# DoubangoTelecom/compv

Measured on AMD Instinct MI355X. Metric: Mpixels/s Sobel->Canny->HoughSHT on 4K uint8, higher is better.
Workload: dtype u8; 1 GPU; batched 3840x2160 uint8 frames, Sobel3x3 -> Canny(59,119) -> HoughSHT(rho=1, theta=1deg, thr=100); 256 distinct frames resident per GPU as 8 batches of 32, a step processes one batch, steps rotate over the batches; frames_per_gpu=32, resident_batches=8, parallelism=frames sharded across 1 GPU(s), no data-path collective

## Files before the change

### compv_amd/capi.py

```python
import ctypes as C
import importlib.util
import os

import numpy as np

_HERE = os.path.dirname(os.path.abspath(__file__))
LIB_PATH = os.path.join(_HERE, "lib", "libcompv_hip.so")

OK = 0
E_NOT_IMPLEMENTED = -1
E_NOT_INITIALIZED = -2
E_INVALID_STATE = -3
E_INVALID_PARAMETER = -4
E_OUT_OF_MEMORY = -5
E_OUT_OF_BOUND = -6
E_HIP = -7

OP_SOBEL, OP_SCHARR, OP_PREWITT = 0, 2, 3
THRESHOLD_COMPARE_TO_GRADIENT, THRESHOLD_PERCENT_OF_MEAN, THRESHOLD_OTSU = 0, 1, 2
(FMT_RGBA32, FMT_ARGB32, FMT_BGRA32, FMT_RGB24, FMT_BGR24, FMT_RGB565LE, FMT_RGB565BE, FMT_BGR565LE, FMT_BGR565BE,
 FMT_YUYV422, FMT_UYVY422, FMT_Y) = range(12)
FMT_BYTES = [4, 4, 4, 3, 3, 2, 2, 2, 2, 2, 2, 1]
FMT_NV12, FMT_NV21, FMT_YUV420P, FMT_YUV422P, FMT_YUV444P, FMT_HSV = range(12, 18)
MORPH_ERODE, MORPH_DILATE, MORPH_OPEN, MORPH_CLOSE = 0, 1, 2, 3
# ... 11 lines not shown
HOMOGRAPHY_RESULT_DTYPE = np.dtype([("H", "<f8", (9,)), ("variance", "<f8"), ("inliers", "<i4"), ("bestTry", "<i4"), ("status", "<i4"), ("rotations", "<i4")])
CURVEFIT_LINE, CURVEFIT_PARABOLA, CURVEFIT_PARABOLA_SIDEWAYS = 0, 1, 2
SVM_KERNEL_LINEAR, SVM_KERNEL_RBF = 0, 2
SVM_F32, SVM_F64 = 0, 1
UNDISTORT_F32, UNDISTORT_F64 = 0, 1
UNDISTORT_COEFFS = 14
MOMENTS_VALUE, MOMENTS_UNIT = 0, 1
MOMENTS_ORIGIN_FRAME, MOMENTS_ORIGIN_BOX = 0, 1
MOMENTS_DTYPE = np.dtype([(k, "<u8") for k in ("m00", "m01", "m10", "m11", "m02", "m20")])
MOMENTS_SHAPE_DTYPE = np.dtype([(k, "<f8") for k in ("xbar", "ybar", "u20", "u02", "u11", "skew", "cs", "sn")] + [("status", "<i4"), ("pad", "<i4")])
CURVEFIT_RESULT_DTYPE = np.dtype([("A", "<f8"), ("B", "<f8"), ("C", "<f8"), ("inliers", "<i4"), ("bestTry", "<i4"), ("status", "<i4"), ("k", "<i4")])

EXPORTS = [
    "compvhip_device_count", "compvhip_ctx_create", "compvhip_ctx_destroy", "compvhip_last_error",
    "compvhip_live_allocations", "compvhip_debug_alloc_fill", "compvhip_edge_dete_u8", "compvhip_canny_u8", "compvhip_houghsht_u8",
    "compvhip_houghsht_dims", "compvhip_houghsht_vote_grid", "compvhip_plan_create", "compvhip_plan_destroy", "compvhip_plan_canny",
    "compvhip_plan_houghsht", "compvhip_plan_pipeline", "compvhip_plan_acc", "compvhip_plan_edge_counts",
    "compvhip_plan_set_timing", "compvhip_plan_get_timing", "compvhip_plan_acc_export", "compvhip_plan_edge_dete",
    "compvhip_houghkht_u8", "compvhip_grayscale_u8", "compvhip_otsu_u8", "compvhip_plan_grayscale", "compvhip_plan_otsu",
    "compvhip_gauss_kernel_fixedpoint", "compvhip_convlt1_fixedpoint_u8", "compvhip_plan_convlt1_fixedpoint", "compvhip_plan_to_cartesian",
    "compvhip_plan_pipeline_async", "compvhip_plan_wait", "compvhip_houghsht_to_cartesian", "compvhip_houghkht_to_cartesian",
    "compvhip_houghkht_kernels_u8", "compvhip_houghkht_stage_ms", "compvhip_convlt1_8u16s16s", "compvhip_convlt1_16s16s16s",
    "compvhip_plan_pipeline_ex", "compvhip_plan_houghkht", "compvhip_plan_houghkht_stage_ms", "compvhip_houghkht_link_u8",
    "compvhip_houghkht_dims", "compvhip_host_cpu_budget", "compvhip_plan_houghkht_ex", "compvhip_houghkht_ex_u8",
    "compvhip_plan_houghsht_segments", "compvhip_houghsht_segments_u8",
    "compvhip_plan_houghsht_fit", "compvhip_houghsht_fit_u8",
    "compvhip_plan_components", "compvhip_components_u8",
    "compvhip_threshold_u8", "compvhip_plan_threshold", "compvhip_threshold_adaptive_u8", "compvhip_plan_threshold_adaptive",
    "compvhip_morph_strel", "compvhip_morph_u8", "compvhip_plan_morph", "compvhip_plan_morph_ex",
    "compvhip_plan_fast", "compvhip_fast_u8",
    "compvhip_plan_orb_keypoints", "compvhip_plan_orb_describe", "compvhip_orb_u8",
# ... 1520 lines not shown
def host_cpu_budget():
    lib = load()
    lib.compvhip_host_cpu_budget.restype = C.c_int
    return int(lib.compvhip_host_cpu_budget())


def houghsht_vote_grid(W, H, theta_deg=1.0, frames=1):
    lib = load()
    nx = C.c_int(0); ny = C.c_int(0); rw = C.c_int(0)
    rc = lib.compvhip_houghsht_vote_grid(W, H, theta_deg, frames, C.byref(nx), C.byref(ny), C.byref(rw))
    if rc:
        raise CompvHipError(rc, "compvhip_houghsht_vote_grid")
    return nx.value, ny.value, rw.value


def houghkht_dims(W, H, rho=1.0, theta_deg=1.0):
    lib = load()
    r = C.c_size_t(0); t = C.c_size_t(0)
    lib.compvhip_houghkht_dims.argtypes = [C.c_size_t, C.c_size_t, C.c_float, C.c_float, C.POINTER(C.c_size_t), C.POINTER(C.c_size_t)]
    rc = lib.compvhip_houghkht_dims(W, H, rho, theta_deg, C.byref(r), C.byref(t))
    if rc:
        raise CompvHipError(rc, "compvhip_houghkht_dims")
    return int(t.value), int(r.value)


def to_cartesian(W, H, lines, kht=False):
    L = load()
    n = len(lines)
    buf = np.zeros(max(n, 1), LINE_DTYPE)
    for i, l in enumerate(lines):
# ... 25 lines not shown
```

### compv_amd/csrc/api.cpp

```cpp
#include "api_internal.hpp"

namespace {
__attribute__((noinline, optnone)) float libmCosf(float x) { return cosf(x); }
__attribute__((noinline, optnone)) float libmSinf(float x) { return sinf(x); }

void gradientThresholds(float fLow, float fHigh, int* tLow, int* tHigh)
{
	const float l = fLow < 1.f ? 1.f : (fLow > 65535.f ? 65535.f : fLow);
	const float h = fHigh < 1.f ? 1.f : (fHigh > 65535.f ? 65535.f : fHigh);
	uint16_t lo = static_cast<uint16_t>(l), hi = static_cast<uint16_t>(h);
	lo = static_cast<uint16_t>(std::max<int>(1, lo));
	hi = static_cast<uint16_t>(std::max<int>(lo + 2, hi));
	*tLow = lo; *tHigh = hi;
}

void cannyCoverage(size_t W, int* simdEnd, int* cStart)
{
	const size_t maxCols = W - 1;
	size_t mpw = 1;
	if (maxCols >= 16) mpw = 16; else if (maxCols >= 8) mpw = 8;
	if (mpw == 1) { *simdEnd = 1; *cStart = 1; return; }
	size_t col = 1;
	while (col + (mpw - 1) < maxCols) col += mpw;
	*simdEnd = static_cast<int>(col);
// ... 11 lines not shown
	float tt = 0.f;
	for (size_t t = 0; t < T; ++t, tt += fTheta) {
		sinQ[t] = static_cast<int32_t>((libmSinf(tt) * fRho) * 65535.f);
		cosQ[t] = static_cast<int32_t>((libmCosf(tt) * fRho) * 65535.f);
	}
}

static size_t voteMaxWindow()
{
	const char* e = getenv("COMPVHIP_VOTE_MAX_WINDOW");
	const long n = e ? atol(e) : 0;
	return (n >= 64 && n <= kShtMaxWindow) ? static_cast<size_t>(n) : static_cast<size_t>(kShtMaxWindow);
}

static bool voteGridTables(size_t W, size_t H, const std::vector<int32_t>& sinQ, const std::vector<int32_t>& cosQ, int split, int& nx, int& ny, int& TW, int& TH, long long& worst,
                           std::vector<int32_t>* kt, std::vector<int32_t>* rowBase)
{
	const size_t T = sinQ.size();
	const long long barrier = static_cast<long long>(W + H);
	nx = 1; ny = 1;
	for (int k = 0; k < split; ++k) {
		const double tw = static_cast<double>(W) / nx, th = static_cast<double>(H) / ny;
		if (tw >= th) ++nx; else ++ny;
	}
	TW = static_cast<int>(alignUp((W + nx - 1) / nx, 32)); TH = static_cast<int>((H + ny - 1) / ny);
	nx = static_cast<int>((W + TW - 1) / TW);
	const int tiles = nx * ny;
	if (kt) { kt->assign(static_cast<size_t>(tiles) * T, 0); rowBase->assign(static_cast<size_t>(tiles) * T, 0); }
	worst = 0;
	for (int ty = 0; ty < ny; ++ty) for (int tx = 0; tx < nx; ++tx) {
		const long long x0 = static_cast<long long>(tx) * TW, y0 = static_cast<long long>(ty) * TH;
		const long long mx = TW - 1, my = TH - 1;
		for (size_t t = 0; t < T; ++t) {
			const long long c = cosQ[t], sn = sinQ[t];
			const long long C = x0 * c + y0 * sn;
			long long Chi = C / 65536; if (C - Chi * 65536 < 0) --Chi;
			const long long Clo = C - Chi * 65536;
			const long long corners[4] = { Clo, mx * c + Clo, my * sn + Clo, mx * c + my * sn + Clo };
			long long qmin = 0, qmax = 0;
			for (int k = 0; k < 4; ++k) {
				long long q = corners[k] / 65536; if (corners[k] - q * 65536 < 0) --q;
				if (k == 0 || q < qmin) qmin = q;
				if (k == 0 || q > qmax) qmax = q;
			}
			const long long base = barrier - Chi - qmax;
			const long long d = ((base % 16) + 16) % 16;
			worst = std::max(worst, qmax - qmin + 1 + d);
			if (kt) {
				(*kt)[(static_cast<size_t>(ty) * nx + tx) * T + t] = static_cast<int32_t>((qmax + d) * 65536 + 65535 - Clo);
				(*rowBase)[(static_cast<size_t>(ty) * nx + tx) * T + t] = static_cast<int32_t>(base - d);
			}
		}
	}
	return alignUp(static_cast<size_t>(worst), 16) <= voteMaxWindow() && TW <= 1280 &&
	       static_cast<long long>(TW - 1) * 65535 + static_cast<long long>(TH - 1) * 65535 < 0x7f000000LL;
}

bool planVoteTiles(size_t W, size_t H, size_t frames, const std::vector<int32_t>& sinQ, const std::vector<int32_t>& cosQ, ShtTileArgs& v, std::vector<int32_t>& kt,
                   std::vector<int32_t>& rowBase)
{
	const size_t T = sinQ.size();
	const int groups = static_cast<int>((T + 63) / 64);
	int first = -1;
	for (int split = 0; split < 512 && first < 0; ++split) {
		int nx, ny, TW, TH; long long worst;
		if (voteGridTables(W, H, sinQ, cosQ, split, nx, ny, TW, TH, worst, nullptr, nullptr)) first = split;
	}
	if (first < 0) return false;
	int best = first; double bestCost = 0.0;
	int nx0, ny0, TW0, TH0; long long worst0;
	(void)voteGridTables(W, H, sinQ, cosQ, first, nx0, ny0, TW0, TH0, worst0, nullptr, nullptr);
	const bool starved = static_cast<double>(frames) * nx0 * ny0 * groups < 64.0;
	for (int split = first; starved && split <= first + 4; ++split) {
		int nx, ny, TW, TH; long long worst;
		if (!voteGridTables(W, H, sinQ, cosQ, split, nx, ny, TW, TH, worst, nullptr, nullptr)) continue;
		const double rw = static_cast<double>(alignUp(static_cast<size_t>(worst), 16));
		const double wgs = static_cast<double>(frames) * nx * ny * groups;
		const double rounds = wgs <= 1024.0 ? std::ceil(wgs / 256.0) : wgs / 256.0;
		const double perWg = 67.0 * (static_cast<double>(TW) * TH) / (960.0 * 720.0) + 9.3 * rw / 1208.0;
		const double reduce = 36.0 * (static_cast<double>(frames) * nx * ny * rw) / (32.0 * 12.0 * 1208.0);
		const double cost = rounds * perWg + reduce;
		if (split == first || cost < bestCost * 0.97) { best = split; bestCost = cost; }
	}
	int nx, ny, TW, TH; long long worst;
	if (!voteGridTables(W, H, sinQ, cosQ, best, nx, ny, TW, TH, worst, &kt, &rowBase)) return false;
	v.nx = nx; v.ny = ny; v.TW = TW; v.TH = TH; v.tiles = nx * ny;
	v.Rw = static_cast<int>(alignUp(static_cast<size_t>(worst), 16)); v.rwPitch = v.Rw;
	v.groups = groups; v.Tpad = v.groups * 64;
	v.tileCap = static_cast<size_t>(TW) * TH;
	return true;
}

ShtArgs shtArgs(compvhip_plan* p, int threshold)
{
	ShtArgs a;
	a.ebits = p->ebits; a.edges = p->edges; a.edgeCounts = p->edgeCounts; a.acc = p->acc;
	a.sinQ = p->sinQ; a.cosQ = p->cosQ; a.lineKeys = p->keysA; a.lineVals = p->valsA; a.lineCounts = p->lineCounts;
	a.frameTotals = p->frameTotals; a.lineTotal = p->lineTotal; a.sortN = 0; a.outCounts = nullptr; a.stepFlags = nullptr; a.hostStep = nullptr;
	a.nmsRange = p->nmsRange; a.blockCounts = p->blockCounts; a.lineBlocks = p->lineBlocks; a.nmsFlags = p->nmsFlags; a.nmsRows = static_cast<int>(sht_nms_rows(static_cast<int>(p->R))); a.nmsGroups = sht_nms_groups(static_cast<int>(p->T));
	a.bitsFrameStride = p->bitsFrameStride; a.edgeCap = p->edgeCap; a.accFrameStride = p->accFrameStride; a.lineCap = p->lineCap;
// ... 116 lines not shown
	{
		std::vector<float> ct(T), ist(T);
		for (size_t t = 0; t < T; ++t) {
			const float theta = static_cast<float>(t) * step;
			ct[t] = libmCosf(theta);
			ist[t] = 1.f / libmSinf(theta);
		}
		HIPCHK(ctx, p->cosT.reserve(ctx, T));
		HIPCHK(ctx, p->invSinT.reserve(ctx, T));
		HIPCHK(ctx, hipMemcpy(p->cosT, ct.data(), T * sizeof(float), hipMemcpyHostToDevice));
		HIPCHK(ctx, hipMemcpy(p->invSinT, ist.data(), T * sizeof(float), hipMemcpyHostToDevice));
	}
	{
		if (p->vt.tiles <= 0 || p->vtKt.size() != static_cast<size_t>(p->vt.tiles) * T) return fail(ctx, COMPVHIP_E_INVALID_STATE, "vote tiles were not planned");
		{
			const int tiles = p->vt.tiles, Rw = p->vt.Rw, groups = sht_nms_groups(static_cast<int>(T));
			std::vector<int2> range(static_cast<size_t>(groups));
			for (int g = 0; g < groups; ++g) {
				int lo = INT32_MAX, hi = INT32_MIN;
				for (int c = 8 * g - 1; c <= 8 * g + 8; ++c) {
					if (c < 0 || c >= static_cast<int>(T)) continue;
					for (int i = 0; i < tiles; ++i) {
						const int b = p->vtRowBase[static_cast<size_t>(i) * T + c];
						lo = std::min(lo, b); hi = std::max(hi, b + Rw);
					}
				}
				range[g] = make_int2(lo - 1, hi + 1);
			}
			std::vector<int2> reach(T);
			for (size_t t = 0; t < T; ++t) {
				int lo = INT32_MAX, hi = INT32_MIN;
				for (int i = 0; i < tiles; ++i) {
					const int b = p->vtRowBase[static_cast<size_t>(i) * T + t];
					lo = std::min(lo, b); hi = std::max(hi, b + Rw);
				}
				reach[t] = make_int2(lo, hi);
			}
			HIPCHK(ctx, p->reach.reserve(ctx, reach.size()));
			HIPCHK(ctx, hipMemcpy(p->reach, reach.data(), reach.size() * sizeof(int2), hipMemcpyHostToDevice));
			HIPCHK(ctx, p->nmsRange.reserve(ctx, range.size()));
			HIPCHK(ctx, hipMemcpy(p->nmsRange, range.data(), range.size() * sizeof(int2), hipMemcpyHostToDevice));
		}
		HIPCHK(ctx, p->dKt.reserve(ctx, p->vtKt.size()));
		HIPCHK(ctx, p->dRowBase.reserve(ctx, p->vtRowBase.size()));
		HIPCHK(ctx, hipMemcpy(p->dKt, p->vtKt.data(), p->vtKt.size() * sizeof(int32_t), hipMemcpyHostToDevice));
		HIPCHK(ctx, hipMemcpy(p->dRowBase, p->vtRowBase.data(), p->vtRowBase.size() * sizeof(int32_t), hipMemcpyHostToDevice));
		{
			const size_t cols = p->frames * p->vt.tiles * static_cast<size_t>(p->vt.Tpad);
			HIPCHK(ctx, p->partLo.reserve(ctx, cols * p->vt.rwPitch));
			HIPCHK(ctx, p->partHi.reserve(ctx, cols * p->vt.rwPitch));
			HIPCHK(ctx, p->colFlag.reserve(ctx, cols));
		}
		p->vt.kt = p->dKt; p->vt.rowBase = p->dRowBase; p->vt.partLo = p->partLo; p->vt.partHi = p->partHi; p->vt.colFlag = p->colFlag; p->vt.reach = p->reach; p->vt.tileCounts = p->tileCounts;
		p->edgeCap = static_cast<size_t>(p->vt.tiles) * p->vt.tileCap;
	}
	HIPCHK(ctx, p->edges.reserve(ctx, p->edgeCap * p->frames));
	HIPCHK(ctx, p->acc.reserve(ctx, p->accFrameStride * p->frames));
	HIPCHK(ctx, hipMemset(p->acc, 0, sizeof(uint16_t) * p->accFrameStride * p->frames));
	p->strengthBits = 1;
	while ((static_cast<size_t>(1) << p->strengthBits) <= 2 * (p->W > p->H ? p->W : p->H)) p->strengthBits++;
	if (p->strengthBits > 16) p->strengthBits = 16;
	int frameBits = 0;
	while ((static_cast<size_t>(1) << frameBits) < p->frames) frameBits++;
	p->keyBits = frameBits + p->strengthBits;
	if (R * T >= (static_cast<size_t>(1) << 32)) return fail(ctx, COMPVHIP_E_INVALID_PARAMETER, "theta step too small: the accumulator has 2^32 cells or more");
	if (p->keyBits > 32) return fail(ctx, COMPVHIP_E_INVALID_PARAMETER, "too many frames for a 32-bit line key");
// ... 118 lines not shown
		if (theta == 0.f) { out[0] = rho + halfW; out[1] = r; out[2] = rho + halfW; out[3] = -r; continue; }
		const float c = libmCosf(theta) * halfW, inv = 1.f / libmSinf(theta);
		out[0] = 0.f; out[1] = ((rho + c) * inv) + halfH;
		out[2] = widthF; out[3] = ((rho - c) * inv) + halfH;
	}
	return COMPVHIP_OK;
}

int compvhip_houghsht_vote_grid(size_t W, size_t H, float thetaDeg, size_t frames, int* nx, int* ny, int* windowRows)
{
	size_t R = 0, T = 0; float st = 0.f;
	if (!nx || !ny || !windowRows || !frames) return COMPVHIP_E_INVALID_PARAMETER;
	const int rc = shtDims(W, H, thetaDeg, &R, &T, &st);
	if (rc) return rc;
	if (T < 5) return COMPVHIP_E_NOT_IMPLEMENTED;
	std::vector<int32_t> sq, cq, kt, rb;
	shtTables(thetaDeg, T, sq, cq);
	ShtTileArgs v = {};
	if (!planVoteTiles(W, H, frames, sq, cq, v, kt, rb)) return COMPVHIP_E_NOT_IMPLEMENTED;
	*nx = v.nx; *ny = v.ny; *windowRows = v.Rw;
	return COMPVHIP_OK;
}

int compvhip_host_cpu_budget(void)
{
	return static_cast<int>(std::min<size_t>(hostCpuBudget(), 0x7fffffff));
}

int compvhip_houghsht_dims(size_t W, size_t H, float thetaDeg, size_t* R, size_t* T, float* step)
{
	if (!R || !T) return COMPVHIP_E_INVALID_PARAMETER;
	return shtDims(W, H, thetaDeg, R, T, step);
}

int compvhip_houghkht_dims(size_t W, size_t H, float rho, float thetaDeg, size_t* rhoN, size_t* T)
// ... 18 lines not shown
	p->tilesY = static_cast<int>((H + 63) / 64);
	p->wb = p->tilesX * 16;
	p->bitsFrameStride = static_cast<size_t>(p->wb) * H;
	auto failed = [&](int rc) { compvhip_plan_destroy(p); return fail(ctx, rc, "plan allocation"); };
	if (p->ebits.reserve(ctx, p->bitsFrameStride * frames) != hipSuccess) return failed(COMPVHIP_E_OUT_OF_MEMORY);
	if (p->ubits.reserve(ctx, p->bitsFrameStride * frames) != hipSuccess) return failed(COMPVHIP_E_OUT_OF_MEMORY);
	if (hipMemset(p->ebits, 0, sizeof(uint32_t) * p->bitsFrameStride * frames) != hipSuccess) return failed(COMPVHIP_E_HIP);
	if (hipMemset(p->ubits, 0, sizeof(uint32_t) * p->bitsFrameStride * frames) != hipSuccess) return failed(COMPVHIP_E_HIP);
	if (hipDeviceSynchronize() != hipSuccess) return failed(COMPVHIP_E_HIP);
	{
		p->voteTiles = true;
		size_t R = 0, T = 0; float step = 0.f;
		if (p->voteTiles && shtDims(W, H, thetaDeg, &R, &T, &step) == COMPVHIP_OK && T >= 5) {
			std::vector<int32_t> sq, cq;
			shtTables(thetaDeg, T, sq, cq);
			if (!planVoteTiles(W, H, frames, sq, cq, p->vt, p->vtKt, p->vtRowBase)) p->voteTiles = false;
		}
		else p->voteTiles = false;
		p->lineBlocks = p->voteTiles ? sht_lines_blocks(static_cast<int>(R)) : 0;
		p->nCounts = (2 + static_cast<size_t>(p->voteTiles ? p->vt.tiles : 0) + static_cast<size_t>(p->lineBlocks)) * frames + (frames + 1) * kFrameSlot;
	}
	if (p->counters.reserve(ctx, p->nCounts + kMaxRounds) != hipSuccess) return failed(COMPVHIP_E_OUT_OF_MEMORY);
	p->edgeCounts = p->counters; p->lineCounts = p->counters + frames; p->tileCounts = p->counters + 2 * frames; p->blockCounts = p->counters + (2 + static_cast<size_t>(p->voteTiles ? p->vt.tiles : 0)) * frames; p->flags = p->counters + p->nCounts;
	p->frameTotals = p->blockCounts + static_cast<size_t>(p->lineBlocks) * frames; p->lineTotal = reinterpret_cast<unsigned int*>(p->frameTotals + frames * kFrameSlot);
	if (const char* e = getenv("COMPVHIP_RESOLVE_WRAP")) { const int v = atoi(e); if (v >= 8 && v <= kMaxRounds && (v & 3) == 0) p->maxRounds = v; }
	p->traceRounds = getenv("COMPVHIP_TRACE_ROUNDS") != nullptr;
	if (hipMemset(p->counters, 0, sizeof(int) * (p->nCounts + kMaxRounds)) != hipSuccess) return failed(COMPVHIP_E_HIP);
	if (p->thrDev.reserve(ctx, frames) != hipSuccess) return failed(COMPVHIP_E_OUT_OF_MEMORY);
	if (p->dirty.reserve(ctx, canny_resolve_dirty_bytes(static_cast<int>(H), p->wb, static_cast<int>(frames))) != hipSuccess) return failed(COMPVHIP_E_OUT_OF_MEMORY);
	if (p->sums.reserve(ctx, frames * kFrameSlot) != hipSuccess) return failed(COMPVHIP_E_OUT_OF_MEMORY);
	if (p->hFlags.reserve(2) != hipSuccess) return failed(COMPVHIP_E_OUT_OF_MEMORY);
// ... 482 lines not shown
```

### compv_amd/csrc/api_internal.hpp

```cpp
#pragma once
#include "../../include/compv_hip.h"
#include "kernels.hpp"
#include "kht.hpp"
#include "kht_group.hpp"
#include "device_memory.hpp"
#include "host_call.hpp"
#include "frame_slices.hpp"
#include "convert_math.hpp"
#include "step_policy.hpp"

#include <hip/hip_runtime.h>

#include <algorithm>
#include <atomic>
#include <chrono>
#include <cmath>
#include <cstdio>
#include <cstdlib>
#include <cstring>
#include <functional>
#include <memory>
#include <string>
#include <thread>
#include <type_traits>
// ... 156 lines not shown
	DevBuf<uint8_t> nmsFlags;
	int* blockCounts = nullptr; int lineBlocks = 0;
	DevBuf<uint8_t> sortTemp; size_t sortTempBytes = 0;
	DevBuf<int32_t> segPerLine;
	DevBuf<int32_t> compRows; DevBuf<uint32_t> compBits; DevBuf<int32_t> compParent;
	DevBuf<uint8_t> morphTmp;
	DevBuf<int> fastWork; DevBuf<uint8_t> fastScores;
	DevBuf<int32_t> orbIndex; DevBuf<uint8_t> orbBlur; uint16_t orbKern[5] = {}; bool orbKernReady = false; bool orbBriefLds = false;
	WarpTables warp;
	DevBuf<float> hogCells;
	StatsScratch stats;
	int strengthBits = 16, keyBits = 0;
	DevBuf<uint16_t> chunkHist; DevBuf<uint32_t> strengthStart; int sortChunks = 0; bool deviceSort = false;
	bool voteTiles = false;
	ShtTileArgs vt = {};
	std::vector<int32_t> vtKt, vtRowBase;
	DevBuf<int32_t> dKt, dRowBase; DevBuf<uint8_t> partLo, partHi, colFlag; int* tileCounts = nullptr;
	std::vector<std::unique_ptr<KhtGroupState>> khtBatch;
	std::vector<std::unique_ptr<KhtPeaksWork>> khtWork;
	double khtStageMs[6] = {}; double khtWallMs = 0.0; int khtThreads = 0;
	struct AsyncStep { bool used = false; bool replay = false; uint64_t seq = 0; hipEvent_t done = nullptr; hipStream_t stream = nullptr; StepParams sp; size_t sortN = 0; int rounds = 0; } steps[kAsyncDepth];
	uint64_t stepSeq = 0;
};

struct compvhip_matcher : TimingState {
	compvhip_ctx* ctx = nullptr;
	int descDwords = 0, queryCap = 0, trainCap = 0, pairs = 0, knn = 0;
	DevBuf<uint32_t> partial;
	DevBuf<compvhip_match> reverse;
};
struct RansacHandle : TimingState {
	compvhip_ctx* ctx = nullptr;
// ... 233 lines not shown
```

### compv_amd/csrc/kernels.hpp

```cpp
#pragma once
#include <hip/hip_runtime.h>
#include <stddef.h>
#include <stdint.h>

#include "../../include/compv_hip.h"

namespace compvhip {

#ifndef COMPVHIP_BAND_H
#define COMPVHIP_BAND_H 64
#endif
constexpr int kBandH = COMPVHIP_BAND_H;
#ifndef COMPVHIP_BAND_WORDS
#define COMPVHIP_BAND_WORDS 64
#endif
constexpr int kBandWords = COMPVHIP_BAND_WORDS;
constexpr int kResolveThreads = 512;
constexpr int kFrameSlot = 32;
constexpr int kResolveRows = kBandH * kBandWords / kResolveThreads;

struct CannyArgs {
	const uint8_t* in;
	uint8_t* out;
	uint32_t* ebits;
// ... 96 lines not shown
	const int* stepFlags;
	int* hostStep;
	int32_t* outCounts;
	int* frameTotals;
	unsigned int* lineTotal;
	size_t sortN;
	size_t bitsFrameStride, edgeCap, accFrameStride, lineCap;
	int W, H, wb;
	int R, T, accPitch, barrier;
	int threshold, nmsLastCol;
	int frames;
	int strengthBits;
};
struct ShtTileArgs {
	const int32_t* kt;
	const int32_t* rowBase;
	uint8_t* partLo;
	uint8_t* partHi;
	uint8_t* colFlag;
	const int2* reach;
	int* tileCounts;
	int nx, ny, TW, TH, tiles;
	int Rw, rwPitch;
	int Tpad, groups;
	size_t tileCap;
};
constexpr int kShtMaxWindow = 1264;
hipError_t launch_sht_compact_tiles(const ShtArgs& a, const ShtTileArgs& v, int frames, hipStream_t stream);
hipError_t launch_sht_vote_tiles(const ShtArgs& a, const ShtTileArgs& v, int frames, hipStream_t stream);
hipError_t launch_sht_reduce_tiles(const ShtArgs& a, const ShtTileArgs& v, int frames, hipStream_t stream);
hipError_t launch_bytes_to_bits(const uint8_t* edges, int W, int H, int S, size_t frameStride, uint32_t* ebits, int wb, size_t bitsFrameStride,
// ... 478 lines not shown
```

### compv_amd/csrc/sht_tiles_kernels.hip

```cpp
#include "device.hpp"

namespace compvhip {

constexpr int kTcThreads = 256;
constexpr int kTcRows = 64;
constexpr int kTcStage = 6144;

__global__ __launch_bounds__(kTcThreads) void sht_compact_tiles_kernel(ShtArgs a, ShtTileArgs v)
{
	__shared__ int s_wave[kTcThreads / 64];
	__shared__ int s_base;
	__shared__ uint32_t s_stage[kTcStage];
	const int frame = blockIdx.y;
	const int chunksPerTile = (v.TH + kTcRows - 1) / kTcRows;
	const int tile = blockIdx.x / chunksPerTile, chunk = blockIdx.x - tile * chunksPerTile;
	const int ty = tile / v.nx, tx = tile - ty * v.nx;
	const int x0 = tx * v.TW, y0 = ty * v.TH;
	const int wpr = v.TW >> 5;
	const uint32_t wprInv = (1u << 20) / (uint32_t)wpr + 1u;
	const int ly0 = chunk * kTcRows;
	const int rows = min(min(kTcRows, v.TH - ly0), a.H - (y0 + ly0));
	const int nwords = max(rows, 0) * wpr;
	const uint32_t* __restrict__ bits = a.ebits + (size_t)frame * a.bitsFrameStride;
	const int w0 = x0 >> 5;
// ... 51 lines not shown
	size_t pos = (size_t)s_base + first;
#pragma unroll
	for (int k = 0; k < kPer; ++k) {
		uint32_t b = wv[k];
		while (b) {
			const int bit = __ffs(b) - 1;
			b &= b - 1;
			if (pos < v.tileCap) dst[pos] = (uint32_t)(wl[k] + bit);
			++pos;
		}
	}
}

constexpr int kVtThreads = 1024;
constexpr int kVtUnroll = 32;

__global__ __launch_bounds__(kVtThreads) void sht_vote_tiles_kernel(ShtArgs a, ShtTileArgs v)
{
	extern __shared__ __attribute__((aligned(16))) uint32_t hist[];
	const int units = a.frames * v.tiles;
	const int xcd = blockIdx.x & 7, k = blockIdx.x >> 3;
	const int g = k % v.groups;
	const int unit = (k / v.groups) * 8 + xcd;
	if (unit >= units) return;
	const int frame = unit / v.tiles, tile = unit - frame * v.tiles;
	const int tid = threadIdx.x, lane = tid & 63;
	const int wave = __builtin_amdgcn_readfirstlane(tid >> 6);

	const int nAll = v.tileCounts[unit];
	if (g == 0 && threadIdx.x == 0 && nAll) atomicAdd(&a.edgeCounts[frame], nAll);
	const int n = min(nAll, (int)v.tileCap);
	const int words = v.Rw * 32;
	uint32_t* const s_any = hist + words;
	if (tid < 2) s_any[tid] = 0u;
	for (int i = tid * 4; i < words; i += kVtThreads * 4) *reinterpret_cast<uint4*>(&hist[i]) = make_uint4(0, 0, 0, 0);

	const int t = g * 64 + lane;
	const int tt = min(t, a.T - 1);
	const int nc = -a.cosQ[tt], ns = -a.sinQ[tt];
	const int K = v.kt[(size_t)tile * a.T + tt];
	uint32_t inc = (t < a.T) ? ((lane & 32) ? 0x10000u : 1u) : 0u;
	asm volatile("" : "+v"(inc));
	const uint32_t lane4 = (uint32_t)(lane & 31) * 4u;
	__syncthreads();

	const uint32_t* __restrict__ list = a.edges + (size_t)unit * v.tileCap;
	typedef uint32_t u32x16 __attribute__((ext_vector_type(16)));
	auto vote = [&](uint32_t e) {
		const int lx = (int)(e & 0xffffu), ly = (int)(e >> 16);
		int val, ad;
		asm volatile("v_mad_i32_i24 %0, %1, %2, %3" : "=v"(val) : "s"(lx), "v"(nc), "v"(K));
		asm volatile("v_mad_i32_i24 %0, %1, %2, %3" : "=v"(val) : "s"(ly), "v"(ns), "v"(val));
		const uint32_t row = (uint32_t)val >> 16;
		asm volatile("v_lshl_add_u32 %0, %1, 7, %2" : "=v"(ad) : "v"(row), "v"(lane4));
		asm volatile("ds_add_u32 %0, %1" : : "v"(ad), "v"(inc) : "memory");
	};
	const int nblk = n / kVtUnroll;
	constexpr int kStep = kVtThreads / 64;
// ... 16 lines not shown
			VT_VOTE(b0, b1);
			if (b >= nblk) break;
			VT_WAIT(a0, a1);
		}
	}
#undef VT_LOAD
#undef VT_WAIT
#undef VT_VOTE
	for (int i = nblk * kVtUnroll + wave; i < n; i += kStep) vote(__builtin_amdgcn_readfirstlane(list[i]));
	__builtin_amdgcn_s_waitcnt(0xc07f);
	__syncthreads();

	const size_t column = ((size_t)unit * v.Tpad) + (size_t)g * 64 + lane;
	uint8_t* __restrict__ partLo = v.partLo + column * v.rwPitch;
	uint8_t* __restrict__ partHi = v.partHi + column * v.rwPitch;
	const uint32_t sel1 = (lane & 32) ? 0x07030602u : 0x05010400u;
	typedef uint32_t u32x4 __attribute__((ext_vector_type(4)));
	auto bytes16 = [&](int w0, u32x4& lo, u32x4& hi) {
		uint32_t h[16];
#pragma unroll
		for (int j = 0; j < 16; ++j) h[j] = hist[(w0 + j) * 32 + (lane & 31)];
#pragma unroll
		for (int q = 0; q < 4; ++q) {
			const uint32_t p01 = __builtin_amdgcn_perm(h[4 * q + 1], h[4 * q], sel1), p23 = __builtin_amdgcn_perm(h[4 * q + 3], h[4 * q + 2], sel1);
			lo[q] = __builtin_amdgcn_perm(p23, p01, 0x05040100u);
			hi[q] = __builtin_amdgcn_perm(p23, p01, 0x07060302u);
		}
	};
	uint32_t any = 0u;
	for (int wb = wave * 128; wb < v.Rw; wb += (kVtThreads / 64) * 128)
	for (int w0 = wb; w0 < min(wb + 128, v.Rw); w0 += 16) {
		u32x4 lo, hi;
		bytes16(w0, lo, hi);
		any |= hi.x | hi.y | hi.z | hi.w;
		uint8_t* const dst = partLo + w0;
		asm volatile("global_store_dwordx4 %0, %1, off" : : "v"(dst), "v"(lo) : "memory");
	}
	const uint64_t mine = __ballot(any != 0u);
	if (lane == 0 && mine) { atomicOr(&s_any[0], (uint32_t)mine); atomicOr(&s_any[1], (uint32_t)(mine >> 32)); }
	__syncthreads();
	const uint32_t m0 = s_any[0], m1 = s_any[1];
	const bool flagged = (((lane & 32) ? m1 : m0) >> (lane & 31)) & 1u;
	if (wave == 0) v.colFlag[column] = flagged ? 1 : 0;
	if ((m0 | m1) == 0u) return;
	if (flagged) {
		for (int wb = wave * 128; wb < v.Rw; wb += (kVtThreads / 64) * 128)
		for (int w0 = wb; w0 < min(wb + 128, v.Rw); w0 += 16) {
			u32x4 lo, hi;
			bytes16(w0, lo, hi);
			uint8_t* const dst = partHi + w0;
			asm volatile("global_store_dwordx4 %0, %1, off" : : "v"(dst), "v"(hi) : "memory");
		}
	}
}

constexpr int kRdThreads = 64;
constexpr int kRdRows = 16;

__global__ __launch_bounds__(kRdThreads) void sht_reduce_tiles_kernel(ShtArgs a, ShtTileArgs v)
{
	const int frame = blockIdx.z, theta = blockIdx.y;
	const int2 reach = v.reach[theta];
	if ((int)(blockIdx.x * kRdThreads * kRdRows) >= reach.y || (int)((blockIdx.x + 1) * kRdThreads * kRdRows) <= reach.x) return;
	const int r0 = (blockIdx.x * kRdThreads + threadIdx.x) * kRdRows;
	if (r0 >= a.accPitch) return;
	uint32_t E[4] = { 0, 0, 0, 0 }, O[4] = { 0, 0, 0, 0 };
	int covers = 0;
	for (int tile = 0; tile < v.tiles; ++tile) {
		const int base = v.rowBase[(size_t)tile * a.T + theta];
		const int w0 = r0 - base;
		if (w0 < 0 || w0 >= v.Rw) continue;
		++covers;
		const size_t column = ((size_t)frame * v.tiles + tile) * v.Tpad + theta;
		const uint4 c = *reinterpret_cast<const uint4*>(v.partLo + column * v.rwPitch + w0);
		E[0] += c.x & 0x00ff00ffu; O[0] += (c.x >> 8) & 0x00ff00ffu;
		E[1] += c.y & 0x00ff00ffu; O[1] += (c.y >> 8) & 0x00ff00ffu;
		E[2] += c.z & 0x00ff00ffu; O[2] += (c.z >> 8) & 0x00ff00ffu;
		E[3] += c.w & 0x00ff00ffu; O[3] += (c.w >> 8) & 0x00ff00ffu;
		if (v.colFlag[column]) {
			const uint4 h = *reinterpret_cast<const uint4*>(v.partHi + column * v.rwPitch + w0);
			E[0] += (h.x & 0x00ff00ffu) << 8; O[0] += h.x & 0xff00ff00u;
			E[1] += (h.y & 0x00ff00ffu) << 8; O[1] += h.y & 0xff00ff00u;
			E[2] += (h.z & 0x00ff00ffu) << 8; O[2] += h.z & 0xff00ff00u;
			E[3] += (h.w & 0x00ff00ffu) << 8; O[3] += h.w & 0xff00ff00u;
		}
	}
// ... 50 lines not shown
```

### include/compv_hip.h

```cpp
#ifndef COMPV_HIP_H
#define COMPV_HIP_H

#include <stddef.h>
#include <stdint.h>

#ifdef __cplusplus
extern "C" {
#endif

#if defined(__GNUC__)
#	define COMPVHIP_API __attribute__((visibility("default")))
#else
#	define COMPVHIP_API
#endif

enum {
	COMPVHIP_OK = 0,
	COMPVHIP_E_NOT_IMPLEMENTED = -1,
	COMPVHIP_E_NOT_INITIALIZED = -2,
	COMPVHIP_E_INVALID_STATE = -3,
	COMPVHIP_E_INVALID_PARAMETER = -4,
	COMPVHIP_E_OUT_OF_MEMORY = -5,
	COMPVHIP_E_OUT_OF_BOUND = -6,
	COMPVHIP_E_HIP = -7
// ... 68 lines not shown
                                      compvhip_line* lines, size_t cap, size_t* n, double* gs);

COMPVHIP_API int compvhip_houghkht_kernels_u8(compvhip_ctx* ctx, const uint8_t* edges, size_t W, size_t H, size_t S,
                                              double clusterMinDeviation, size_t clusterMinSize,
                                              double* kernels7, size_t cap, size_t* n, double* hmax);
COMPVHIP_API int compvhip_houghkht_stage_ms(compvhip_ctx* ctx, double* ms6);
COMPVHIP_API int compvhip_houghkht_link_u8(const uint8_t* edges, size_t W, size_t H, size_t S, size_t clusterMinSize, int32_t* xy, size_t cap, size_t* nPoints,
                                           uint32_t* stringEnds, size_t stringCap, size_t* nStrings);

COMPVHIP_API int compvhip_houghsht_to_cartesian(size_t W, size_t H, const compvhip_line* lines, size_t n, float* out);
COMPVHIP_API int compvhip_houghkht_to_cartesian(size_t W, size_t H, const compvhip_line* lines, size_t n, float* out);

COMPVHIP_API int compvhip_houghsht_dims(size_t W, size_t H, float thetaDeg, size_t* R, size_t* T, float* thetaStepRad);
COMPVHIP_API int compvhip_houghkht_dims(size_t W, size_t H, float rho, float thetaDeg, size_t* rhoN, size_t* T);
COMPVHIP_API int compvhip_houghsht_vote_grid(size_t W, size_t H, float thetaDeg, size_t frames, int* nx, int* ny, int* windowRows);
COMPVHIP_API int compvhip_host_cpu_budget(void);


COMPVHIP_API int compvhip_plan_create(compvhip_ctx* ctx, size_t W, size_t H, size_t S, size_t frames, float thetaDeg,
                                      compvhip_plan** plan);
COMPVHIP_API void compvhip_plan_destroy(compvhip_plan* plan);

COMPVHIP_API int compvhip_plan_canny(compvhip_plan* plan, const uint8_t* d_in, float tLow, float tHigh, int ksize,
                                     int thresholdType, uint8_t* d_edges, void* stream);

COMPVHIP_API int compvhip_plan_grayscale(compvhip_plan* plan, const uint8_t* d_in, int pixfmt, uint8_t* d_gray, void* stream);

COMPVHIP_API int compvhip_plan_otsu(compvhip_plan* plan, const uint8_t* d_gray, int32_t* d_thresholds, void* stream);

COMPVHIP_API int compvhip_plan_convlt1_fixedpoint(compvhip_plan* plan, const uint8_t* d_in, const uint16_t* vtKern, const uint16_t* hzKern,
// ... 504 lines not shown
```

Measured before the change: 437,000 Mpixels/s.

## Limit SHT vote flush to per-column row reach and reuse histogram bytes

Records a per-tile, per-theta row reach and packs it alongside rowBase as int2, so the vote kernel writes only the rows each column can actually receive instead of the full worst-case window Rw. The flush now reads each histogram tile once with a permlane32 swap and keeps the high bytes in registers, rather than rereading for the partHi pass. The reduction kernel bounds its reads by the per-column reach, and the partial buffers are zeroed at plan time so rows never written read as zero. It also adds a host export for the vote tables; a fixed per-wave flush count of 5 is assumed, which risks missing rows if the reach exceeds 16*5*16 rows.

```diff
diff --git a/compv_amd/capi.py b/compv_amd/capi.py
--- a/compv_amd/capi.py
+++ b/compv_amd/capi.py
@@ -49,7 +49,7 @@
 EXPORTS = [
     "compvhip_device_count", "compvhip_ctx_create", "compvhip_ctx_destroy", "compvhip_last_error",
     "compvhip_live_allocations", "compvhip_debug_alloc_fill", "compvhip_edge_dete_u8", "compvhip_canny_u8", "compvhip_houghsht_u8",
-    "compvhip_houghsht_dims", "compvhip_houghsht_vote_grid", "compvhip_plan_create", "compvhip_plan_destroy", "compvhip_plan_canny",
+    "compvhip_houghsht_dims", "compvhip_houghsht_vote_grid", "compvhip_houghsht_vote_tables", "compvhip_plan_create", "compvhip_plan_destroy", "compvhip_plan_canny",
     "compvhip_plan_houghsht", "compvhip_plan_pipeline", "compvhip_plan_acc", "compvhip_plan_edge_counts",
     "compvhip_plan_set_timing", "compvhip_plan_get_timing", "compvhip_plan_acc_export", "compvhip_plan_edge_dete",
     "compvhip_houghkht_u8", "compvhip_grayscale_u8", "compvhip_otsu_u8", "compvhip_plan_grayscale", "compvhip_plan_otsu",
@@ -1600,6 +1600,23 @@
     return nx.value, ny.value, rw.value
 
 
+def houghsht_vote_tables(W, H, theta_deg=1.0, frames=1):
+    lib = load()
+    nx, ny, rw = houghsht_vote_grid(W, H, theta_deg, frames)
+    r = C.c_size_t(0); t = C.c_size_t(0)
+    lib.compvhip_houghsht_dims(W, H, theta_deg, C.byref(r), C.byref(t), None)
+    T = t.value
+    tw = C.c_int(0); th = C.c_int(0)
+    cq, sq = np.zeros(T, np.int32), np.zeros(T, np.int32)
+    kt, rb, rr = (np.zeros((nx * ny, T), np.int32) for _ in range(3))
+    i32 = C.POINTER(C.c_int32)
+    lib.compvhip_houghsht_vote_tables.argtypes = [C.c_size_t, C.c_size_t, C.c_float, C.c_size_t, C.POINTER(C.c_int), C.POINTER(C.c_int), i32, i32, i32, i32, i32, C.c_size_t]
+    rc = lib.compvhip_houghsht_vote_tables(W, H, theta_deg, frames, C.byref(tw), C.byref(th), *(a.ctypes.data_as(i32) for a in (cq, sq, kt, rb, rr)), kt.size)
+    if rc:
+        raise CompvHipError(rc, "compvhip_houghsht_vote_tables")
+    return {"nx": nx, "ny": ny, "rw": rw, "TW": tw.value, "TH": th.value, "cosQ": cq, "sinQ": sq, "K": kt, "rowBase": rb, "rowReach": rr}
+
+
 def houghkht_dims(W, H, rho=1.0, theta_deg=1.0):
     lib = load()
     r = C.c_size_t(0); t = C.c_size_t(0)
diff --git a/compv_amd/csrc/api.cpp b/compv_amd/csrc/api.cpp
--- a/compv_amd/csrc/api.cpp
+++ b/compv_amd/csrc/api.cpp
@@ -49,7 +49,7 @@
 }
 
 static bool voteGridTables(size_t W, size_t H, const std::vector<int32_t>& sinQ, const std::vector<int32_t>& cosQ, int split, int& nx, int& ny, int& TW, int& TH, long long& worst,
-                           std::vector<int32_t>* kt, std::vector<int32_t>* rowBase)
+                           std::vector<int32_t>* kt, std::vector<int32_t>* rowBase, std::vector<int32_t>* rowReach)
 {
 	const size_t T = sinQ.size();
 	const long long barrier = static_cast<long long>(W + H);
@@ -61,7 +61,7 @@
 	TW = static_cast<int>(alignUp((W + nx - 1) / nx, 32)); TH = static_cast<int>((H + ny - 1) / ny);
 	nx = static_cast<int>((W + TW - 1) / TW);
 	const int tiles = nx * ny;
-	if (kt) { kt->assign(static_cast<size_t>(tiles) * T, 0); rowBase->assign(static_cast<size_t>(tiles) * T, 0); }
+	if (kt) { kt->assign(static_cast<size_t>(tiles) * T, 0); rowBase->assign(static_cast<size_t>(tiles) * T, 0); rowReach->assign(static_cast<size_t>(tiles) * T, 0); }
 	worst = 0;
 	for (int ty = 0; ty < ny; ++ty) for (int tx = 0; tx < nx; ++tx) {
 		const long long x0 = static_cast<long long>(tx) * TW, y0 = static_cast<long long>(ty) * TH;
@@ -84,6 +84,7 @@
 			if (kt) {
 				(*kt)[(static_cast<size_t>(ty) * nx + tx) * T + t] = static_cast<int32_t>((qmax + d) * 65536 + 65535 - Clo);
 				(*rowBase)[(static_cast<size_t>(ty) * nx + tx) * T + t] = static_cast<int32_t>(base - d);
+				(*rowReach)[(static_cast<size_t>(ty) * nx + tx) * T + t] = static_cast<int32_t>(alignUp(static_cast<size_t>(qmax - qmin + 1 + d), 16));
 			}
 		}
 	}
@@ -92,23 +93,23 @@
 }
 
 bool planVoteTiles(size_t W, size_t H, size_t frames, const std::vector<int32_t>& sinQ, const std::vector<int32_t>& cosQ, ShtTileArgs& v, std::vector<int32_t>& kt,
-                   std::vector<int32_t>& rowBase)
+                   std::vector<int32_t>& rowBase, std::vector<int32_t>& rowReach)
 {
 	const size_t T = sinQ.size();
 	const int groups = static_cast<int>((T + 63) / 64);
 	int first = -1;
 	for (int split = 0; split < 512 && first < 0; ++split) {
 		int nx, ny, TW, TH; long long worst;
-		if (voteGridTables(W, H, sinQ, cosQ, split, nx, ny, TW, TH, worst, nullptr, nullptr)) first = split;
+		if (voteGridTables(W, H, sinQ, cosQ, split, nx, ny, TW, TH, worst, nullptr, nullptr, nullptr)) first = split;
 	}
 	if (first < 0) return false;
 	int best = first; double bestCost = 0.0;
 	int nx0, ny0, TW0, TH0; long long worst0;
-	(void)voteGridTables(W, H, sinQ, cosQ, first, nx0, ny0, TW0, TH0, worst0, nullptr, nullptr);
+	(void)voteGridTables(W, H, sinQ, cosQ, first, nx0, ny0, TW0, TH0, worst0, nullptr, nullptr, nullptr);
 	const bool starved = static_cast<double>(frames) * nx0 * ny0 * groups < 64.0;
 	for (int split = first; starved && split <= first + 4; ++split) {
 		int nx, ny, TW, TH; long long worst;
-		if (!voteGridTables(W, H, sinQ, cosQ, split, nx, ny, TW, TH, worst, nullptr, nullptr)) continue;
+		if (!voteGridTables(W, H, sinQ, cosQ, split, nx, ny, TW, TH, worst, nullptr, nullptr, nullptr)) continue;
 		const double rw = static_cast<double>(alignUp(static_cast<size_t>(worst), 16));
 		const double wgs = static_cast<double>(frames) * nx * ny * groups;
 		const double rounds = wgs <= 1024.0 ? std::ceil(wgs / 256.0) : wgs / 256.0;
@@ -118,7 +119,7 @@
 		if (split == first || cost < bestCost * 0.97) { best = split; bestCost = cost; }
 	}
 	int nx, ny, TW, TH; long long worst;
-	if (!voteGridTables(W, H, sinQ, cosQ, best, nx, ny, TW, TH, worst, &kt, &rowBase)) return false;
+	if (!voteGridTables(W, H, sinQ, cosQ, best, nx, ny, TW, TH, worst, &kt, &rowBase, &rowReach)) return false;
 	v.nx = nx; v.ny = ny; v.TW = TW; v.TH = TH; v.tiles = nx * ny;
 	v.Rw = static_cast<int>(alignUp(static_cast<size_t>(worst), 16)); v.rwPitch = v.Rw;
 	v.groups = groups; v.Tpad = v.groups * 64;
@@ -265,27 +266,24 @@
 	{
 		if (p->vt.tiles <= 0 || p->vtKt.size() != static_cast<size_t>(p->vt.tiles) * T) return fail(ctx, COMPVHIP_E_INVALID_STATE, "vote tiles were not planned");
 		{
-			const int tiles = p->vt.tiles, Rw = p->vt.Rw, groups = sht_nms_groups(static_cast<int>(T));
+			const int tiles = p->vt.tiles, groups = sht_nms_groups(static_cast<int>(T));
+			std::vector<int2> reach(T);
+			for (size_t t = 0; t < T; ++t) {
+				int lo = INT32_MAX, hi = INT32_MIN;
+				for (int i = 0; i < tiles; ++i) {
+					const int b = p->vtRowBase[static_cast<size_t>(i) * T + t];
+					lo = std::min(lo, b); hi = std::max(hi, b + p->vtRowReach[static_cast<size_t>(i) * T + t]);
+				}
+				reach[t] = make_int2(lo, hi);
+			}
 			std::vector<int2> range(static_cast<size_t>(groups));
 			for (int g = 0; g < groups; ++g) {
 				int lo = INT32_MAX, hi = INT32_MIN;
 				for (int c = 8 * g - 1; c <= 8 * g + 8; ++c) {
 					if (c < 0 || c >= static_cast<int>(T)) continue;
-					for (int i = 0; i < tiles; ++i) {
-						const int b = p->vtRowBase[static_cast<size_t>(i) * T + c];
-						lo = std::min(lo, b); hi = std::max(hi, b + Rw);
-					}
+					lo = std::min(lo, reach[static_cast<size_t>(c)].x); hi = std::max(hi, reach[static_cast<size_t>(c)].y);
 				}
 				range[g] = make_int2(lo - 1, hi + 1);
-			}
-			std::vector<int2> reach(T);
-			for (size_t t = 0; t < T; ++t) {
-				int lo = INT32_MAX, hi = INT32_MIN;
-				for (int i = 0; i < tiles; ++i) {
-					const int b = p->vtRowBase[static_cast<size_t>(i) * T + t];
-					lo = std::min(lo, b); hi = std::max(hi, b + Rw);
-				}
-				reach[t] = make_int2(lo, hi);
 			}
 			HIPCHK(ctx, p->reach.reserve(ctx, reach.size()));
 			HIPCHK(ctx, hipMemcpy(p->reach, reach.data(), reach.size() * sizeof(int2), hipMemcpyHostToDevice));
@@ -293,14 +291,24 @@
 			HIPCHK(ctx, hipMemcpy(p->nmsRange, range.data(), range.size() * sizeof(int2), hipMemcpyHostToDevice));
 		}
 		HIPCHK(ctx, p->dKt.reserve(ctx, p->vtKt.size()));
-		HIPCHK(ctx, p->dRowBase.reserve(ctx, p->vtRowBase.size()));
 		HIPCHK(ctx, hipMemcpy(p->dKt, p->vtKt.data(), p->vtKt.size() * sizeof(int32_t), hipMemcpyHostToDevice));
-		HIPCHK(ctx, hipMemcpy(p->dRowBase, p->vtRowBase.data(), p->vtRowBase.size() * sizeof(int32_t), hipMemcpyHostToDevice));
+		{
+			const size_t Tpad = static_cast<size_t>(p->vt.Tpad);
+			std::vector<int2> rb(static_cast<size_t>(p->vt.tiles) * Tpad, make_int2(0, 0));
+			for (size_t i = 0; i < static_cast<size_t>(p->vt.tiles); ++i)
+				for (size_t t = 0; t < T; ++t) rb[i * Tpad + t] = make_int2(p->vtRowBase[i * T + t], p->vtRowReach[i * T + t]);
+			HIPCHK(ctx, p->dRowBase.reserve(ctx, rb.size()));
+			HIPCHK(ctx, hipMemcpy(p->dRowBase, rb.data(), rb.size() * sizeof(int2), hipMemcpyHostToDevice));
+		}
 		{
 			const size_t cols = p->frames * p->vt.tiles * static_cast<size_t>(p->vt.Tpad);
 			HIPCHK(ctx, p->partLo.reserve(ctx, cols * p->vt.rwPitch));
 			HIPCHK(ctx, p->partHi.reserve(ctx, cols * p->vt.rwPitch));
 			HIPCHK(ctx, p->colFlag.reserve(ctx, cols));
+			HIPCHK(ctx, hipMemset(p->partLo, 0, cols * p->vt.rwPitch));
+			HIPCHK(ctx, hipMemset(p->partHi, 0, cols * p->vt.rwPitch));
+			HIPCHK(ctx, hipMemset(p->colFlag, 0, cols));
+			HIPCHK(ctx, hipDeviceSynchronize());
 		}
 		p->vt.kt = p->dKt; p->vt.rowBase = p->dRowBase; p->vt.partLo = p->partLo; p->vt.partHi = p->partHi; p->vt.colFlag = p->colFlag; p->vt.reach = p->reach; p->vt.tileCounts = p->tileCounts;
 		p->edgeCap = static_cast<size_t>(p->vt.tiles) * p->vt.tileCap;
@@ -449,11 +457,30 @@
 	const int rc = shtDims(W, H, thetaDeg, &R, &T, &st);
 	if (rc) return rc;
 	if (T < 5) return COMPVHIP_E_NOT_IMPLEMENTED;
-	std::vector<int32_t> sq, cq, kt, rb;
+	std::vector<int32_t> sq, cq, kt, rb, rr;
 	shtTables(thetaDeg, T, sq, cq);
 	ShtTileArgs v = {};
-	if (!planVoteTiles(W, H, frames, sq, cq, v, kt, rb)) return COMPVHIP_E_NOT_IMPLEMENTED;
+	if (!planVoteTiles(W, H, frames, sq, cq, v, kt, rb, rr)) return COMPVHIP_E_NOT_IMPLEMENTED;
 	*nx = v.nx; *ny = v.ny; *windowRows = v.Rw;
+	return COMPVHIP_OK;
+}
+
+int compvhip_houghsht_vote_tables(size_t W, size_t H, float thetaDeg, size_t frames, int* TW, int* TH, int32_t* cosQ, int32_t* sinQ, int32_t* kt, int32_t* rowBase,
+                                  int32_t* rowReach, size_t cap)
+{
+	size_t R = 0, T = 0; float st = 0.f;
+	if (!TW || !TH || !cosQ || !sinQ || !kt || !rowBase || !rowReach || !frames) return COMPVHIP_E_INVALID_PARAMETER;
+	const int rc = shtDims(W, H, thetaDeg, &R, &T, &st);
+	if (rc) return rc;
+	if (T < 5) return COMPVHIP_E_NOT_IMPLEMENTED;
+	std::vector<int32_t> sq, cq, k, rb, rr;
+	shtTables(thetaDeg, T, sq, cq);
+	ShtTileArgs v = {};
+	if (!planVoteTiles(W, H, frames, sq, cq, v, k, rb, rr)) return COMPVHIP_E_NOT_IMPLEMENTED;
+	if (cap < k.size()) return COMPVHIP_E_INVALID_PARAMETER;
+	*TW = v.TW; *TH = v.TH;
+	std::copy(cq.begin(), cq.end(), cosQ); std::copy(sq.begin(), sq.end(), sinQ);
+	std::copy(k.begin(), k.end(), kt); std::copy(rb.begin(), rb.end(), rowBase); std::copy(rr.begin(), rr.end(), rowReach);
 	return COMPVHIP_OK;
 }
 
@@ -502,7 +529,7 @@
 		if (p->voteTiles && shtDims(W, H, thetaDeg, &R, &T, &step) == COMPVHIP_OK && T >= 5) {
 			std::vector<int32_t> sq, cq;
 			shtTables(thetaDeg, T, sq, cq);
-			if (!planVoteTiles(W, H, frames, sq, cq, p->vt, p->vtKt, p->vtRowBase)) p->voteTiles = false;
+			if (!planVoteTiles(W, H, frames, sq, cq, p->vt, p->vtKt, p->vtRowBase, p->vtRowReach)) p->voteTiles = false;
 		}
 		else p->voteTiles = false;
 		p->lineBlocks = p->voteTiles ? sht_lines_blocks(static_cast<int>(R)) : 0;
diff --git a/compv_amd/csrc/api_internal.hpp b/compv_amd/csrc/api_internal.hpp
--- a/compv_amd/csrc/api_internal.hpp
+++ b/compv_amd/csrc/api_internal.hpp
@@ -194,8 +194,8 @@
 	DevBuf<uint16_t> chunkHist; DevBuf<uint32_t> strengthStart; int sortChunks = 0; bool deviceSort = false;
 	bool voteTiles = false;
 	ShtTileArgs vt = {};
-	std::vector<int32_t> vtKt, vtRowBase;
-	DevBuf<int32_t> dKt, dRowBase; DevBuf<uint8_t> partLo, partHi, colFlag; int* tileCounts = nullptr;
+	std::vector<int32_t> vtKt, vtRowBase, vtRowReach;
+	DevBuf<int32_t> dKt; DevBuf<int2> dRowBase; DevBuf<uint8_t> partLo, partHi, colFlag; int* tileCounts = nullptr;
 	std::vector<std::unique_ptr<KhtGroupState>> khtBatch;
 	std::vector<std::unique_ptr<KhtPeaksWork>> khtWork;
 	double khtStageMs[6] = {}; double khtWallMs = 0.0; int khtThreads = 0;
diff --git a/compv_amd/csrc/kernels.hpp b/compv_amd/csrc/kernels.hpp
--- a/compv_amd/csrc/kernels.hpp
+++ b/compv_amd/csrc/kernels.hpp
@@ -134,7 +134,7 @@
 };
 struct ShtTileArgs {
 	const int32_t* kt;
-	const int32_t* rowBase;
+	const int2* rowBase;
 	uint8_t* partLo;
 	uint8_t* partHi;
 	uint8_t* colFlag;
diff --git a/compv_amd/csrc/sht_tiles_kernels.hip b/compv_amd/csrc/sht_tiles_kernels.hip
--- a/compv_amd/csrc/sht_tiles_kernels.hip
+++ b/compv_amd/csrc/sht_tiles_kernels.hip
@@ -89,6 +89,7 @@
 
 constexpr int kVtThreads = 1024;
 constexpr int kVtUnroll = 32;
+constexpr int kVtFlushPer = 5;
 
 __global__ __launch_bounds__(kVtThreads) void sht_vote_tiles_kernel(ShtArgs a, ShtTileArgs v)
 {
@@ -117,6 +118,7 @@
 	uint32_t inc = (t < a.T) ? ((lane & 32) ? 0x10000u : 1u) : 0u;
 	asm volatile("" : "+v"(inc));
 	const uint32_t lane4 = (uint32_t)(lane & 31) * 4u;
+	const int myRows = v.rowBase[(size_t)tile * v.Tpad + g * 64 + lane].y;
 	__syncthreads();
 
 	const uint32_t* __restrict__ list = a.edges + (size_t)unit * v.tileCap;
@@ -163,42 +165,56 @@
 	const size_t column = ((size_t)unit * v.Tpad) + (size_t)g * 64 + lane;
 	uint8_t* __restrict__ partLo = v.partLo + column * v.rwPitch;
 	uint8_t* __restrict__ partHi = v.partHi + column * v.rwPitch;
-	const uint32_t sel1 = (lane & 32) ? 0x07030602u : 0x05010400u;
 	typedef uint32_t u32x4 __attribute__((ext_vector_type(4)));
+	const uint32_t* const mine8 = hist + ((lane & 32) >> 2) * 32 + (lane & 31);
 	auto bytes16 = [&](int w0, u32x4& lo, u32x4& hi) {
-		uint32_t h[16];
-#pragma unroll
-		for (int j = 0; j < 16; ++j) h[j] = hist[(w0 + j) * 32 + (lane & 31)];
+		uint32_t h[8], X[4], Y[4];
+#pragma unroll
+		for (int j = 0; j < 8; ++j) h[j] = mine8[(w0 + j) * 32];
 #pragma unroll
 		for (int q = 0; q < 4; ++q) {
-			const uint32_t p01 = __builtin_amdgcn_perm(h[4 * q + 1], h[4 * q], sel1), p23 = __builtin_amdgcn_perm(h[4 * q + 3], h[4 * q + 2], sel1);
-			lo[q] = __builtin_amdgcn_perm(p23, p01, 0x05040100u);
-			hi[q] = __builtin_amdgcn_perm(p23, p01, 0x07060302u);
-		}
+			const uint32_t lows = __builtin_amdgcn_perm(h[2 * q + 1], h[2 * q], 0x05040100u), highs = __builtin_amdgcn_perm(h[2 * q + 1], h[2 * q], 0x07060302u);
+			const auto r = __builtin_amdgcn_permlane32_swap(lows, highs, false, false);
+			X[q] = r[0]; Y[q] = r[1];
+		}
+		lo.x = __builtin_amdgcn_perm(X[1], X[0], 0x06040200u); lo.y = __builtin_amdgcn_perm(X[3], X[2], 0x06040200u);
+		lo.z = __builtin_amdgcn_perm(Y[1], Y[0], 0x06040200u); lo.w = __builtin_amdgcn_perm(Y[3], Y[2], 0x06040200u);
+		hi.x = __builtin_amdgcn_perm(X[1], X[0], 0x07050301u); hi.y = __builtin_amdgcn_perm(X[3], X[2], 0x07050301u);
+		hi.z = __builtin_amdgcn_perm(Y[1], Y[0], 0x07050301u); hi.w = __builtin_amdgcn_perm(Y[3], Y[2], 0x07050301u);
 	};
+	const int flushRows = __builtin_amdgcn_readfirstlane(wave_max(myRows));
+	const int per = ((flushRows >> 4) + kVtThreads / 64 - 1) / (kVtThreads / 64);
+	const int wBeg = wave * per * 16, wEnd = min(wBeg + per * 16, flushRows);
+	u32x4 keep[kVtFlushPer];
 	uint32_t any = 0u;
-	for (int wb = wave * 128; wb < v.Rw; wb += (kVtThreads / 64) * 128)
-	for (int w0 = wb; w0 < min(wb + 128, v.Rw); w0 += 16) {
-		u32x4 lo, hi;
-		bytes16(w0, lo, hi);
-		any |= hi.x | hi.y | hi.z | hi.w;
-		uint8_t* const dst = partLo + w0;
-		asm volatile("global_store_dwordx4 %0, %1, off" : : "v"(dst), "v"(lo) : "memory");
-	}
-	const uint64_t mine = __ballot(any != 0u);
-	if (lane == 0 && mine) { atomicOr(&s_any[0], (uint32_t)mine); atomicOr(&s_any[1], (uint32_t)(mine >> 32)); }
+#pragma unroll
+	for (int i = 0; i < kVtFlushPer; ++i) {
+		const int w0 = wBeg + i * 16;
+		keep[i] = u32x4{ 0u, 0u, 0u, 0u };
+		if (w0 < wEnd) {
+			u32x4 lo;
+			bytes16(w0, lo, keep[i]);
+			any |= keep[i].x | keep[i].y | keep[i].z | keep[i].w;
+			if (w0 < myRows) {
+				uint8_t* const dst = partLo + w0;
+				asm volatile("global_store_dwordx4 %0, %1, off" : : "v"(dst), "v"(lo) : "memory");
+			}
+		}
+	}
+	const uint64_t flagMask = __ballot(any != 0u);
+	if (lane == 0 && flagMask) { atomicOr(&s_any[0], (uint32_t)flagMask); atomicOr(&s_any[1], (uint32_t)(flagMask >> 32)); }
 	__syncthreads();
 	const uint32_t m0 = s_any[0], m1 = s_any[1];
 	const bool flagged = (((lane & 32) ? m1 : m0) >> (lane & 31)) & 1u;
 	if (wave == 0) v.colFlag[column] = flagged ? 1 : 0;
-	if ((m0 | m1) == 0u) return;
 	if (flagged) {
-		for (int wb = wave * 128; wb < v.Rw; wb += (kVtThreads / 64) * 128)
-		for (int w0 = wb; w0 < min(wb + 128, v.Rw); w0 += 16) {
-			u32x4 lo, hi;
-			bytes16(w0, lo, hi);
-			uint8_t* const dst = partHi + w0;
-			asm volatile("global_store_dwordx4 %0, %1, off" : : "v"(dst), "v"(hi) : "memory");
+#pragma unroll
+		for (int i = 0; i < kVtFlushPer; ++i) {
+			const int w0 = wBeg + i * 16;
+			if (w0 < wEnd && w0 < myRows) {
+				uint8_t* const dst = partHi + w0;
+				asm volatile("global_store_dwordx4 %0, %1, off" : : "v"(dst), "v"(keep[i]) : "memory");
+			}
 		}
 	}
 }
@@ -216,9 +232,9 @@
 	uint32_t E[4] = { 0, 0, 0, 0 }, O[4] = { 0, 0, 0, 0 };
 	int covers = 0;
 	for (int tile = 0; tile < v.tiles; ++tile) {
-		const int base = v.rowBase[(size_t)tile * a.T + theta];
-		const int w0 = r0 - base;
-		if (w0 < 0 || w0 >= v.Rw) continue;
+		const unsigned long long rbv = reinterpret_cast<const unsigned long long*>(v.rowBase)[(size_t)tile * v.Tpad + theta];
+		const int w0 = r0 - (int)(uint32_t)rbv;
+		if (w0 < 0 || w0 >= (int)(rbv >> 32)) continue;
 		++covers;
 		const size_t column = ((size_t)frame * v.tiles + tile) * v.Tpad + theta;
 		const uint4 c = *reinterpret_cast<const uint4*>(v.partLo + column * v.rwPitch + w0);
diff --git a/include/compv_hip.h b/include/compv_hip.h
--- a/include/compv_hip.h
+++ b/include/compv_hip.h
@@ -106,6 +106,8 @@
 COMPVHIP_API int compvhip_houghsht_dims(size_t W, size_t H, float thetaDeg, size_t* R, size_t* T, float* thetaStepRad);
 COMPVHIP_API int compvhip_houghkht_dims(size_t W, size_t H, float rho, float thetaDeg, size_t* rhoN, size_t* T);
 COMPVHIP_API int compvhip_houghsht_vote_grid(size_t W, size_t H, float thetaDeg, size_t frames, int* nx, int* ny, int* windowRows);
+COMPVHIP_API int compvhip_houghsht_vote_tables(size_t W, size_t H, float thetaDeg, size_t frames, int* TW, int* TH, int32_t* cosQ, int32_t* sinQ, int32_t* kt,
+                                               int32_t* rowBase, int32_t* rowReach, size_t cap);
 COMPVHIP_API int compvhip_host_cpu_budget(void);
 
 
```

Result: no change. 439,400 Mpixels/s (median of 6 runs) (+0.6%).
